# INET-RC/GeoMX

Measured on AMD Instinct MI355X. Metric: samples/sec (whole node), higher is better.
Workload: dtype bf16; 1 GPU; model=geomx_cnn, input=3x224x224, global_batch=512, per_gpu_batch=512, parallelism=dp1, sync_mode=dist_sync, optimizer=sgd_mom

## Files before the change

geomx_amd/csrc/fc.hip:

```cpp

#include <hip/hip_runtime.h>

#include <cstdint>

typedef unsigned short bf16_t;
typedef __attribute__((ext_vector_type(8))) short bf16x8;

#define FC_C 32
#define FC_THREADS 256
#define FC_PERM_HW 128
#define FC_PERM_LD 129

__device__ __forceinline__ bf16_t fc_f2bf(float f) {
  union { float f; unsigned int u; } cv;
  cv.f = f;
  if ((cv.u & 0x7FFFFFFFu) > 0x7F800000u)
    return (bf16_t)((cv.u >> 16) | 0x0040u);
  const unsigned int lsb = (cv.u >> 16) & 1;
  return (bf16_t)((cv.u + 0x7FFFu + lsb) >> 16);
}

__global__ __launch_bounds__(FC_THREADS) void k_fc_w_permute_bf16(
    const float* __restrict__ w, bf16_t* __restrict__ wp, int HW) {
  __shared__ float tile[FC_C * FC_PERM_LD];
  const int t = threadIdx.x;
  const int hw0 = blockIdx.x * FC_PERM_HW;
  const long long o = blockIdx.y;
  const float* src = w + o * FC_C * HW;
  {
    const int hw = t & (FC_PERM_HW - 1), c0 = t >> 7;
    if (hw0 + hw < HW) {
      float v[FC_C / 2];
#pragma unroll
      for (int i = 0; i < FC_C / 2; ++i)
        v[i] = src[(long long)(c0 + 2 * i) * HW + hw0 + hw];
#pragma unroll
      for (int i = 0; i < FC_C / 2; ++i)
        tile[(c0 + 2 * i) * FC_PERM_LD + hw] = v[i];
    }
  }
  __syncthreads();
  bf16_t* dst = wp + o * HW * FC_C;
  const int cg = t & 3;
#pragma unroll
  for (int p = 0; p < FC_PERM_HW / (FC_THREADS / 4); ++p) {
    const int hw = p * (FC_THREADS / 4) + (t >> 2);
    if (hw0 + hw < HW) {
      union { bf16x8 v; bf16_t e[8]; } pk;
#pragma unroll
      for (int j = 0; j < 8; ++j)
        pk.e[j] = fc_f2bf(tile[(cg * 8 + j) * FC_PERM_LD + hw]);
      *reinterpret_cast<bf16x8*>(dst + (long long)(hw0 + hw) * FC_C +
                                 cg * 8) = pk.v;
    }
  }
}

__global__ __launch_bounds__(FC_THREADS) void k_fc_w_unpermute_f32(
    const bf16_t* __restrict__ gp, float* __restrict__ g, int HW) {
  __shared__ float tile[FC_C * FC_PERM_LD];
  const int t = threadIdx.x;
  const int hw0 = blockIdx.x * FC_PERM_HW;
  const long long o = blockIdx.y;
  const bf16_t* src = gp + o * HW * FC_C;
  const int cg = t & 3;
#pragma unroll
  for (int p = 0; p < FC_PERM_HW / (FC_THREADS / 4); ++p) {
    const int hw = p * (FC_THREADS / 4) + (t >> 2);
    if (hw0 + hw < HW) {
      union { bf16x8 v; bf16_t e[8]; } pk;
      pk.v = *reinterpret_cast<const bf16x8*>(
          src + (long long)(hw0 + hw) * FC_C + cg * 8);
#pragma unroll
      for (int j = 0; j < 8; ++j) {
        union { unsigned int u; float f; } cv;
        cv.u = (unsigned int)pk.e[j] << 16;
        tile[(cg * 8 + j) * FC_PERM_LD + hw] = cv.f;
      }
    }
  }
  __syncthreads();
  float* dst = g + o * FC_C * HW;
  const int hw = t & (FC_PERM_HW - 1), c0 = t >> 7;
  if (hw0 + hw < HW) {
#pragma unroll
    for (int i = 0; i < FC_C / 2; ++i)
      dst[(long long)(c0 + 2 * i) * HW + hw0 + hw] =
          tile[(c0 + 2 * i) * FC_PERM_LD + hw];
  }
}

#define FC_FLAT_LD 130
__global__ __launch_bounds__(FC_THREADS) void k_fc_flatten_nchw(
    const bf16_t* __restrict__ x, bf16_t* __restrict__ y, int HW) {
  __shared__ bf16_t tile[FC_C * FC_FLAT_LD];
  const int t = threadIdx.x;
  const int hw0 = blockIdx.x * FC_PERM_HW;
  const long long n = blockIdx.y;
  const bf16_t* src = x + n * HW * FC_C;
  const int cg = t & 3;
#pragma unroll
  for (int p = 0; p < FC_PERM_HW / (FC_THREADS / 4); ++p) {
    const int hw = p * (FC_THREADS / 4) + (t >> 2);
    if (hw0 + hw < HW) {
      union { bf16x8 v; bf16_t e[8]; } pk;
      pk.v = *reinterpret_cast<const bf16x8*>(
          src + (long long)(hw0 + hw) * FC_C + cg * 8);
#pragma unroll
      for (int j = 0; j < 8; ++j)
        tile[(cg * 8 + j) * FC_FLAT_LD + hw] = pk.e[j];
    }
  }
  __syncthreads();
  const int wave = t >> 6, lane = t & 63;
#pragma unroll
  for (int i = 0; i < FC_C / 4; ++i) {
    const int c = wave * (FC_C / 4) + i;
    const long long row = (n * FC_C + c) * HW + hw0;
    const int par = (int)(row & 1);
    const bf16_t* trow = tile + c * FC_FLAT_LD;
    bf16_t* dst = y + row;
    const int e0 = 2 * lane - par, e1 = e0 + 1;
    const bool ok0 = e0 >= 0 && hw0 + e0 < HW;
    const bool ok1 = hw0 + e1 < HW;
    if (ok0 && ok1) {
      const unsigned v = (unsigned)trow[e0] | ((unsigned)trow[e1] << 16);
      *reinterpret_cast<unsigned*>(dst + e0) = v;
    } else if (ok0) {
      dst[e0] = trow[e0];
    } else if (ok1) {
      dst[e1] = trow[e1];
    }
    if (par && lane == 0 && hw0 + FC_PERM_HW - 1 < HW)
      dst[FC_PERM_HW - 1] = trow[FC_PERM_HW - 1];
  }
}

extern "C" {

static bool fc_geometry_ok(long long rows, int C, int HW) {
  return C == FC_C && rows > 0 && rows <= 65535 && HW > 0 &&
         HW <= (1 << 24);
}

int geops_fc_w_permute_bf16(const float* w, bf16_t* wp, int O, int C, int HW,
                            hipStream_t s) {
  if (!fc_geometry_ok(O, C, HW)) return -1;
  hipLaunchKernelGGL(k_fc_w_permute_bf16,
                     dim3((HW + FC_PERM_HW - 1) / FC_PERM_HW, O),
                     dim3(FC_THREADS), 0, s, w, wp, HW);
  return 0;
}

int geops_fc_w_unpermute_f32(const bf16_t* gp, float* g, int O, int C, int HW,
                             hipStream_t s) {
  if (!fc_geometry_ok(O, C, HW)) return -1;
  hipLaunchKernelGGL(k_fc_w_unpermute_f32,
                     dim3((HW + FC_PERM_HW - 1) / FC_PERM_HW, O),
                     dim3(FC_THREADS), 0, s, gp, g, HW);
  return 0;
}

int geops_fc_flatten_nchw(const bf16_t* x, bf16_t* y, int N, int C, int HW,
                          hipStream_t s) {
  if (!fc_geometry_ok(N, C, HW)) return -1;
  hipLaunchKernelGGL(k_fc_flatten_nchw,
                     dim3((HW + FC_PERM_HW - 1) / FC_PERM_HW, N),
                     dim3(FC_THREADS), 0, s, x, y, HW);
  return 0;
}

}
```

geomx_amd/csrc/geops.cpp:

```cpp

#include <torch/extension.h>

#include <ATen/cuda/CUDAContext.h>
#include <hip/hip_runtime.h>

#include <cstdint>

extern "C" {
void geops_quantize_2bit(const float*, float*, uint32_t*, long long, float,
                         hipStream_t);
void geops_dequantize_2bit(const uint32_t*, float*, long long, float,
                           hipStream_t);
void geops_bsc_momentum(const float*, float*, float*, float, long long,
                        hipStream_t);
void geops_bsc_pack(const float*, float*, float*, float*, int*, long long*,
                    float, long long, long long, float, bool, hipStream_t);
void geops_bsc_pull_pack(const float*, float*, int*, long long*, long long,
                         long long, float, hipStream_t);
int geops_bsc_fused(const float*, float*, float*, float*, int*, const float*,
                    unsigned long long*, float, long long, long long, float,
                    hipStream_t);
void geops_bsc_unpack(const float*, const int*, float*, long long, long long,
                      bool, hipStream_t);
void geops_dgt_contribution(const float*, float*, long long, int, int,
                            hipStream_t);
void geops_quantize_4bit(const float*, float*, uint8_t*, float*, long long,
                         int, int, bool, hipStream_t);
void geops_dequantize_4bit(const uint8_t*, const float*, float*, long long,
                           int, hipStream_t);
void geops_sgd_update(float*, const float*, float, float, float, long long,
                      hipStream_t);
void geops_sgd_mom_update(float*, const float*, float*, float, float, float,
                          float, long long, hipStream_t);
void geops_adam_update(float*, const float*, float*, float*, float, float,
                       float, float, float, float, long long, hipStream_t);
void geops_dcasgd_update(float*, const float*, float*, float*, float, float,
                         float, float, float, long long, bool, hipStream_t);
void geops_rmsprop_update(float*, const float*, float*, float, float, float,
                          float, float, long long, hipStream_t);
void geops_adagrad_update(float*, const float*, float*, float, float, float,
                          float, long long, hipStream_t);
void geops_signsgd_update(float*, const float*, float, float, float,
                          long long, hipStream_t);
void geops_signum_update(float*, const float*, float*, float, float, float,
                         float, long long, hipStream_t);
void geops_rsp_merge(const long long*, const long long*, const long long*,
                     const float*, long long*, float*, long long, long long,
                     hipStream_t);
void geops_rsp_scatter(const long long*, const float*, float*, long long,
                       long long, long long, bool, hipStream_t);
void geops_rsp_sgd_update(const long long*, const float*, float*, float,
                          float, float, long long, long long, long long,
                          hipStream_t);
void geops_rsp_sgd_mom_update(const long long*, const float*, float*, float*,
                              float, float, float, float, long long,
                              long long, long long, hipStream_t);
void geops_rsp_adam_update(const long long*, const float*, float*, float*,
                           float*, float, float, float, float, float, float,
                           long long, long long, long long, hipStream_t);
void geops_rsp_adagrad_update(const long long*, const float*, float*, float*,
                              float, float, float, float, long long,
                              long long, long long, hipStream_t);
void geops_relu_maxpool2_fwd(const unsigned short*, unsigned short*, uint8_t*,
                             long long, int, int, int, hipStream_t);
void geops_relu_maxpool2_bwd(const unsigned short*, const uint8_t*,
                             unsigned short*, long long, int, int, int,
                             hipStream_t);
int geops_conv5_nhwc(const unsigned short*, const unsigned short*,
                     const float*, unsigned short*, int, int, int, int, int,
                     int, int, int, hipStream_t);
int geops_conv5_pool_nhwc(const unsigned short*, const unsigned short*,
                          const float*, unsigned short*, uint8_t*, int, int,
                          int, int, int, int, int, hipStream_t);
int geops_conv5_pool_nwg_nhwc(const unsigned short*, const unsigned short*,
                              const float*, unsigned short*, uint8_t*, int,
                              int, int, int, int, int, int, int, hipStream_t);
void geops_pad_ch3to4_nhwc(const void*, unsigned short*, long long, int,
                           hipStream_t);
int geops_conv5_pack_frags(const float*, long long, const long long*,
                           unsigned short*, long long, const long long*,
                           unsigned short*, long long, hipStream_t);
int geops_conv5_wrw16_nhwc(const unsigned short*, const unsigned short*,
                           float*, int, int, int, int, int, int, int, int,
                           hipStream_t);
int geops_conv5_wrw4_nhwc(const unsigned short*, const unsigned short*,
                          float*, int, int, int, int, int, int, int, int,
                          hipStream_t);
int geops_conv5_wrw_unpool_nhwc(const unsigned short*, const unsigned short*,
                                const uint8_t*, float*, int, int, int, int,
                                int, int, int, int, hipStream_t);
int geops_conv5_dgrad_unpool_nhwc(const unsigned short*, const uint8_t*,
                                  const unsigned short*, unsigned short*,
                                  int, int, int, int, int, int, int,
                                  hipStream_t);
int geops_conv5_direct_nhwc(const unsigned short*, const unsigned short*,
                            const float*, unsigned short*, int, int, int, int,
                            int, int, int, hipStream_t);
int geops_conv5_dgrad_nwg_nhwc(const unsigned short*, const uint8_t*,
                               const unsigned short*, unsigned short*, int,
                               int, int, int, int, int, int, int,
                               hipStream_t);
int geops_fc_w_permute_bf16(const float*, unsigned short*, int, int, int,
                            hipStream_t);
int geops_fc_w_unpermute_f32(const unsigned short*, float*, int, int, int,
                             hipStream_t);
int geops_fc_flatten_nchw(const unsigned short*, unsigned short*, int, int,
                          int, hipStream_t);
void geops_tr16_probe(const unsigned short*, unsigned short*, hipStream_t);
void geops_tr16_probe2(const unsigned short*, const int*, unsigned short*,
                       hipStream_t);
}

namespace {

hipStream_t cur_stream() {
  return (hipStream_t)at::cuda::getCurrentCUDAStream().stream();
}

void launch_check(const char* what) {
  const hipError_t e = hipGetLastError();
  TORCH_CHECK(e == hipSuccess, what, ": kernel launch failed: ",
              hipGetErrorString(e));
}

void check_f32(const torch::Tensor& t, const char* name) {
  TORCH_CHECK(t.is_cuda(), name, " must be a GPU tensor");
  TORCH_CHECK(t.is_contiguous(), name, " must be contiguous");
  TORCH_CHECK(t.scalar_type() == torch::kFloat32, name, " must be fp32");
  TORCH_CHECK(((uintptr_t)t.data_ptr() & 15) == 0, name,
              " must be 16-byte aligned");
}

void quantize_2bit(torch::Tensor grad, torch::Tensor residual,
                   torch::Tensor out, double thr) {
  check_f32(grad, "grad");
  check_f32(residual, "residual");
  TORCH_CHECK(out.scalar_type() == torch::kInt32 && out.is_contiguous());
  const long long n = grad.numel();
  TORCH_CHECK(residual.numel() == n);
  TORCH_CHECK(out.numel() == (n + 15) / 16);
  geops_quantize_2bit(grad.data_ptr<float>(), residual.data_ptr<float>(),
                      (uint32_t*)out.data_ptr<int32_t>(), n, (float)thr,
                      cur_stream());
  launch_check("quantize_2bit");
}

void dequantize_2bit(torch::Tensor packed, torch::Tensor out, double thr) {
  check_f32(out, "out");
  TORCH_CHECK(packed.scalar_type() == torch::kInt32 && packed.is_contiguous());
  const long long n = out.numel();
  TORCH_CHECK(packed.numel() >= (n + 15) / 16);
  geops_dequantize_2bit((const uint32_t*)packed.data_ptr<int32_t>(),
                        out.data_ptr<float>(), n, (float)thr, cur_stream());
  launch_check("dequantize_2bit");
}

void bsc_momentum(torch::Tensor g, torch::Tensor u, torch::Tensor v,
                  double mu) {
  check_f32(g, "g"); check_f32(u, "u"); check_f32(v, "v");
  const long long n = g.numel();
  TORCH_CHECK(u.numel() == n && v.numel() == n);
  geops_bsc_momentum(g.data_ptr<float>(), u.data_ptr<float>(),
                     v.data_ptr<float>(), (float)mu, n, cur_stream());
  launch_check("bsc_momentum");
}

torch::Tensor make_workspace(const torch::Tensor& like) {
  return torch::empty({2049}, torch::TensorOptions()
                                  .dtype(torch::kInt64)
                                  .device(like.device()));
}

void bsc_pack(torch::Tensor v, torch::Tensor u, torch::Tensor vals,
              torch::Tensor idx, double boundary, double placeholder) {
  check_f32(v, "v"); check_f32(u, "u"); check_f32(vals, "vals");
  TORCH_CHECK(idx.scalar_type() == torch::kInt32 && idx.is_contiguous());
  TORCH_CHECK(vals.numel() == idx.numel());
  auto ws = make_workspace(v);
  geops_bsc_pack(v.data_ptr<float>(), v.data_ptr<float>(),
                 u.data_ptr<float>(), vals.data_ptr<float>(),
                 idx.data_ptr<int32_t>(), (long long*)ws.data_ptr<int64_t>(),
                 (float)boundary, v.numel(), vals.numel(),
                 (float)placeholder, true, cur_stream());
  launch_check("bsc_pack");
}

bool bsc_compress_fused(torch::Tensor g, torch::Tensor u, torch::Tensor v,
                        torch::Tensor vals, torch::Tensor idx,
                        torch::Tensor boundary, double mu,
                        double placeholder) {
// ... 282 lines not shown
  const int rc = geops_conv5_direct_nhwc(
      (const unsigned short*)in.data_ptr(),
      (const unsigned short*)w_frags.data_ptr(), nullptr,
      (unsigned short*)out.data_ptr(), (int)N, (int)Hi, (int)Wi, (int)Ho,
      (int)Wo, (int)CI, (int)CO, cur_stream());
  TORCH_CHECK(rc == 0, "conv5_direct_nhwc: unsupported geometry CI=", CI,
              " CO=", CO, " Hi=", Hi, " Wi=", Wi);
  launch_check("conv5_direct_nhwc");
}

void conv5_dgrad_nwg_nhwc(torch::Tensor in, torch::Tensor mask,
                          torch::Tensor w_frags, torch::Tensor out,
                          int64_t N, int64_t Hi, int64_t Wi, int64_t Ho,
                          int64_t Wo, int64_t CI, int64_t CO, int64_t n_wg) {
  const bool pooled = mask.defined() && mask.numel() > 0;
  TORCH_CHECK(in.is_cuda() && w_frags.is_cuda() && out.is_cuda());
  TORCH_CHECK(in.scalar_type() == torch::kBFloat16 &&
              w_frags.scalar_type() == torch::kBFloat16 &&
              out.scalar_type() == torch::kBFloat16);
  TORCH_CHECK(Hi >= 10 && Wi >= 10 && n_wg >= 1 && n_wg <= 65536,
              "conv5_dgrad_nwg_nhwc: bad size or n_wg");
  if (pooled) {
    TORCH_CHECK(mask.is_cuda() && mask.scalar_type() == torch::kUInt8);
    TORCH_CHECK(in.numel() == N * ((Hi - 8) / 2) * ((Wi - 8) / 2) * CI &&
                    mask.numel() == in.numel(),
                "conv5_dgrad_nwg_nhwc: pooled gradient / mask size mismatch");
  } else {
    TORCH_CHECK(in.numel() == N * (Hi - 8) * (Wi - 8) * CI,
                "conv5_dgrad_nwg_nhwc: gradient size mismatch");
  }
  TORCH_CHECK(out.numel() == N * Ho * Wo * CO &&
                  w_frags.numel() == 25 * 64 * 8,
              "conv5_dgrad_nwg_nhwc: output / weight size mismatch");
  const int rc = geops_conv5_dgrad_nwg_nhwc(
      (const unsigned short*)in.data_ptr(),
      pooled ? mask.data_ptr<uint8_t>() : nullptr,
      (const unsigned short*)w_frags.data_ptr(),
      (unsigned short*)out.data_ptr(), (int)N, (int)Hi, (int)Wi, (int)Ho,
      (int)Wo, (int)CI, (int)CO, (int)n_wg, cur_stream());
  TORCH_CHECK(rc == 0, "conv5_dgrad_nwg_nhwc: unsupported geometry CI=", CI,
              " CO=", CO, " Hi=", Hi, " Wi=", Wi);
  launch_check("conv5_dgrad_nwg_nhwc");
}


void check_fc_operand(const torch::Tensor& t, torch::ScalarType dtype,
                      int64_t numel, const char* name) {
  TORCH_CHECK(t.is_cuda(), name, " must be a GPU tensor");
  TORCH_CHECK(t.is_contiguous(), name, " must be contiguous");
  TORCH_CHECK(t.scalar_type() == dtype, name, " has the wrong dtype");
  TORCH_CHECK(t.numel() == numel, name, " has ", t.numel(),
              " elements, expected ", numel);
  if (dtype != torch::kFloat32)
    TORCH_CHECK(((uintptr_t)t.data_ptr() & 15) == 0, name,
                " must be 16-byte aligned");
}

torch::Tensor fc_w_permute_bf16(torch::Tensor w, int64_t O, int64_t C,
                                int64_t HW) {
  check_fc_operand(w, torch::kFloat32, O * C * HW, "weight");
  auto wp = torch::empty({O, HW * C}, w.options().dtype(torch::kBFloat16));
  const int rc = geops_fc_w_permute_bf16(
      w.data_ptr<float>(), (unsigned short*)wp.data_ptr(), (int)O, (int)C,
      (int)HW, cur_stream());
  TORCH_CHECK(rc == 0, "fc_w_permute_bf16: unsupported geometry O=", O,
              " C=", C, " HW=", HW);
  launch_check("fc_w_permute_bf16");
  return wp;
}

torch::Tensor fc_w_unpermute_f32(torch::Tensor gp, int64_t O, int64_t C,
                                 int64_t HW) {
  check_fc_operand(gp, torch::kBFloat16, O * C * HW, "permuted gradient");
  auto g = torch::empty({O, C * HW}, gp.options().dtype(torch::kFloat32));
  const int rc = geops_fc_w_unpermute_f32(
      (const unsigned short*)gp.data_ptr(), g.data_ptr<float>(), (int)O,
      (int)C, (int)HW, cur_stream());
  TORCH_CHECK(rc == 0, "fc_w_unpermute_f32: unsupported geometry O=", O,
              " C=", C, " HW=", HW);
  launch_check("fc_w_unpermute_f32");
  return g;
}

torch::Tensor fc_flatten_nchw(torch::Tensor x, int64_t N, int64_t C,
                              int64_t HW) {
  check_fc_operand(x, torch::kBFloat16, N * C * HW, "x");
  auto y = torch::empty({N, C * HW}, x.options());
  const int rc = geops_fc_flatten_nchw(
      (const unsigned short*)x.data_ptr(), (unsigned short*)y.data_ptr(),
      (int)N, (int)C, (int)HW, cur_stream());
  TORCH_CHECK(rc == 0, "fc_flatten_nchw: unsupported geometry N=", N,
              " C=", C, " HW=", HW);
  launch_check("fc_flatten_nchw");
  return y;
}

void pad_ch3to4_nhwc(torch::Tensor in, torch::Tensor out, int64_t npix) {
  TORCH_CHECK(in.is_cuda() && out.is_cuda());
  TORCH_CHECK(out.scalar_type() == torch::kBFloat16);
  const bool fp32 = in.scalar_type() == torch::kFloat32;
  TORCH_CHECK(fp32 || in.scalar_type() == torch::kBFloat16);
  geops_pad_ch3to4_nhwc(in.data_ptr(), (unsigned short*)out.data_ptr(),
                        npix, fp32 ? 1 : 0, cur_stream());
  launch_check("pad_ch3to4_nhwc");
}

std::vector<torch::Tensor> conv5_pack_frags(torch::Tensor weight,
                                            torch::Tensor idx0,
                                            c10::optional<torch::Tensor> idx1) {
  TORCH_CHECK(weight.is_cuda() && weight.is_contiguous() &&
                  weight.scalar_type() == torch::kFloat32,
              "conv5_pack_frags: weight must be contiguous fp32 on the GPU");
  const bool two = idx1.has_value() && idx1->defined();
  auto check_idx = [&](const torch::Tensor& t) {
    TORCH_CHECK(t.is_cuda() && t.is_contiguous() &&
                    t.scalar_type() == torch::kInt64 &&
                    t.device() == weight.device() && t.numel() > 0 &&
                    t.numel() % 8 == 0,
                "conv5_pack_frags: index tables are contiguous int64 on the "
                "weight's device, a multiple of 8 long");
  };
  check_idx(idx0);
  if (two) check_idx(*idx1);
  const auto opts = weight.options().dtype(torch::kBFloat16);
  std::vector<torch::Tensor> out;
  out.push_back(torch::empty({idx0.numel()}, opts));
  if (two) out.push_back(torch::empty({idx1->numel()}, opts));
  const int rc = geops_conv5_pack_frags(
      weight.data_ptr<float>(), (long long)weight.numel(),
      (const long long*)idx0.data_ptr<int64_t>(),
      (unsigned short*)out[0].data_ptr(), (long long)idx0.numel(),
      two ? (const long long*)idx1->data_ptr<int64_t>() : nullptr,
      two ? (unsigned short*)out[1].data_ptr() : nullptr,
      two ? (long long)idx1->numel() : 0LL, cur_stream());
  TORCH_CHECK(rc == 0, "conv5_pack_frags: bad table sizes");
  launch_check("conv5_pack_frags");
  return out;
}

void sgd_update(torch::Tensor w, torch::Tensor g, double lr, double wd,
                double rescale) {
  check_f32(w, "w"); check_f32(g, "g");
  TORCH_CHECK(w.numel() == g.numel());
  geops_sgd_update(w.data_ptr<float>(), g.data_ptr<float>(), (float)lr,
                   (float)wd, (float)rescale, w.numel(), cur_stream());
  launch_check("sgd_update");
}

void sgd_mom_update(torch::Tensor w, torch::Tensor g, torch::Tensor mom,
                    double lr, double momentum, double wd, double rescale) {
  check_f32(w, "w"); check_f32(g, "g"); check_f32(mom, "mom");
  geops_sgd_mom_update(w.data_ptr<float>(), g.data_ptr<float>(),
                       mom.data_ptr<float>(), (float)lr, (float)momentum,
                       (float)wd, (float)rescale, w.numel(), cur_stream());
  launch_check("sgd_mom_update");
}

void adam_update(torch::Tensor w, torch::Tensor g, torch::Tensor m,
                 torch::Tensor v, int64_t t, double lr, double beta1,
                 double beta2, double eps, double wd, double rescale) {
  check_f32(w, "w"); check_f32(g, "g"); check_f32(m, "m"); check_f32(v, "v");
  const double lr_t =
      lr * std::sqrt(1.0 - std::pow(beta2, (double)t)) /
      (1.0 - std::pow(beta1, (double)t));
  geops_adam_update(w.data_ptr<float>(), g.data_ptr<float>(),
                    m.data_ptr<float>(), v.data_ptr<float>(), (float)lr_t,
// ... 116 lines not shown
  launch_check("rsp_scatter");
}

void rsp_sgd_update(torch::Tensor w, torch::Tensor ids, torch::Tensor merged,
                    double lr, double wd, double rescale) {
  check_rsp_rows(w, ids, merged);
  geops_rsp_sgd_update(i64p(ids), merged.data_ptr<float>(),
                       w.data_ptr<float>(), (float)lr, (float)wd,
                       (float)rescale, ids.numel(), w.size(0), w.size(1),
                       cur_stream());
  launch_check("rsp_sgd_update");
}

void rsp_sgd_mom_update(torch::Tensor w, torch::Tensor ids,
                        torch::Tensor merged, torch::Tensor mom, double lr,
                        double momentum, double wd, double rescale) {
  check_rsp_rows(w, ids, merged);
  check_rsp_state(mom, w, "mom");
  geops_rsp_sgd_mom_update(i64p(ids), merged.data_ptr<float>(),
                           w.data_ptr<float>(), mom.data_ptr<float>(),
                           (float)lr, (float)momentum, (float)wd,
                           (float)rescale, ids.numel(), w.size(0), w.size(1),
                           cur_stream());
  launch_check("rsp_sgd_mom_update");
}

void rsp_adam_update(torch::Tensor w, torch::Tensor ids, torch::Tensor merged,
                     torch::Tensor m, torch::Tensor v, int64_t t, double lr,
                     double beta1, double beta2, double eps, double wd,
                     double rescale) {
  check_rsp_rows(w, ids, merged);
  check_rsp_state(m, w, "m"); check_rsp_state(v, w, "v");
  const double lr_t =
      lr * std::sqrt(1.0 - std::pow(beta2, (double)t)) /
      (1.0 - std::pow(beta1, (double)t));
  geops_rsp_adam_update(i64p(ids), merged.data_ptr<float>(),
                        w.data_ptr<float>(), m.data_ptr<float>(),
                        v.data_ptr<float>(), (float)lr_t, (float)beta1,
                        (float)beta2, (float)eps, (float)wd, (float)rescale,
                        ids.numel(), w.size(0), w.size(1), cur_stream());
  launch_check("rsp_adam_update");
}

void rsp_adagrad_update(torch::Tensor w, torch::Tensor ids,
                        torch::Tensor merged, torch::Tensor h, double lr,
                        double eps, double wd, double rescale) {
  check_rsp_rows(w, ids, merged);
  check_rsp_state(h, w, "h");
  geops_rsp_adagrad_update(i64p(ids), merged.data_ptr<float>(),
                           w.data_ptr<float>(), h.data_ptr<float>(),
                           (float)lr, (float)eps, (float)wd, (float)rescale,
                           ids.numel(), w.size(0), w.size(1), cur_stream());
  launch_check("rsp_adagrad_update");
}

}

PYBIND11_MODULE(TORCH_EXTENSION_NAME, m) {
  m.doc() = "geomx_amd gfx950 kernel library";
  m.def("quantize_2bit", &quantize_2bit);
  m.def("dequantize_2bit", &dequantize_2bit);
  m.def("bsc_momentum", &bsc_momentum);
  m.def("bsc_pack", &bsc_pack);
  m.def("bsc_pull_pack", &bsc_pull_pack);
  m.def("bsc_compress_fused", &bsc_compress_fused);
  m.def("bsc_unpack", &bsc_unpack);
  m.def("dgt_contribution", &dgt_contribution);
  m.def("quantize_4bit", &quantize_4bit);
  m.def("dequantize_4bit", &dequantize_4bit);
  m.def("conv5_nhwc", &conv5_nhwc);
  m.def("pad_ch3to4_nhwc", &pad_ch3to4_nhwc);
  m.def("conv5_pack_frags", &conv5_pack_frags, py::arg("weight"),
        py::arg("idx0"), py::arg("idx1") = py::none());
  m.def("conv5_wrw_nhwc", &conv5_wrw_nhwc);
  m.def("conv5_wrw_unpool_nhwc", &conv5_wrw_unpool_nhwc);
  m.def("conv5_dgrad_unpool_nhwc", &conv5_dgrad_unpool_nhwc);
  m.def("conv5_direct_nhwc", &conv5_direct_nhwc);
  m.def("conv5_dgrad_nwg_nhwc", &conv5_dgrad_nwg_nhwc);
  m.def("conv5_pool_nhwc", &conv5_pool_nhwc);
  m.def("conv5_pool_nwg_nhwc", &conv5_pool_nwg_nhwc);
  m.def("fc_w_permute_bf16", &fc_w_permute_bf16);
  m.def("fc_w_unpermute_f32", &fc_w_unpermute_f32);
  m.def("fc_flatten_nchw", &fc_flatten_nchw);
  m.def("tr16_probe2", [](torch::Tensor in, torch::Tensor addr,
                          torch::Tensor out) {
    TORCH_CHECK(in.is_cuda() && addr.is_cuda() && out.is_cuda());
    TORCH_CHECK(in.numel() == 512 && addr.numel() == 64 &&
                out.numel() == 256);
    TORCH_CHECK(addr.scalar_type() == torch::kInt32);
    geops_tr16_probe2((const unsigned short*)in.data_ptr(),
                      addr.data_ptr<int32_t>(),
                      (unsigned short*)out.data_ptr(), cur_stream());
    launch_check("tr16_probe2");
  });
  m.def("tr16_probe", [](torch::Tensor in, torch::Tensor out) {
    TORCH_CHECK(in.is_cuda() && out.is_cuda());
    TORCH_CHECK(in.numel() == 64 && out.numel() == 256);
    geops_tr16_probe((const unsigned short*)in.data_ptr(),
                     (unsigned short*)out.data_ptr(), cur_stream());
    launch_check("tr16_probe");
  });
  m.def("relu_maxpool2_fwd", &relu_maxpool2_fwd);
  m.def("relu_maxpool2_bwd", &relu_maxpool2_bwd);
  m.def("sgd_update", &sgd_update);
  m.def("sgd_mom_update", &sgd_mom_update);
  m.def("adam_update", &adam_update);
  m.def("dcasgd_update", &dcasgd_update);
  m.def("rmsprop_update", &rmsprop_update);
  m.def("adagrad_update", &adagrad_update);
  m.def("signsgd_update", &signsgd_update);
  m.def("signum_update", &signum_update);
  m.def("rsp_merge", &rsp_merge);
  m.def("rsp_scatter", &rsp_scatter);
  m.def("rsp_sgd_update", &rsp_sgd_update);
  m.def("rsp_sgd_mom_update", &rsp_sgd_mom_update);
  m.def("rsp_adam_update", &rsp_adam_update);
  m.def("rsp_adagrad_update", &rsp_adagrad_update);
}
```

geomx_amd/ops/fc.py:

```python

from __future__ import annotations

import torch
import torch.nn.functional as F

from . import native_available

FC_CHANNELS = 32


def supported(C: int, O: int, N: int, HW: int) -> bool:
    return (C == FC_CHANNELS and 0 < O <= 65535 and N > 0
            and 0 < HW <= (1 << 24))


def native_route(x: torch.Tensor, weight: torch.Tensor) -> bool:
    if not (x.is_cuda and x.dim() == 4 and native_available()):
        return False
    if torch.is_autocast_enabled("cuda"):
        if torch.get_autocast_dtype("cuda") != torch.bfloat16 or \
                x.dtype not in (torch.bfloat16, torch.float32):
            return False
    elif x.dtype != torch.bfloat16:
        return False
    N, C, H, W = x.shape
    if not supported(C, weight.shape[0], N, H * W):
        return False
    if weight.dtype != torch.float32 or not weight.is_contiguous() \
            or weight.shape[1] != C * H * W:
        return False
    return x.stride() == (H * W * C, 1, W * C, C)


class _FlattenLinearFn(torch.autograd.Function):

    @staticmethod
    def forward(ctx, x, weight, bias):
        from geomx_amd import _geops
        N, C, H, W = x.shape
        xf = x.detach().to(torch.bfloat16).permute(0, 2, 3, 1) \
            .reshape(N, H * W * C)
        with torch.autocast("cuda", enabled=False):
            y = F.linear(_geops.fc_flatten_nchw(xf, N, C, H * W),
                         weight.detach().to(torch.bfloat16),
                         None if bias is None
                         else bias.detach().to(torch.bfloat16))
        ctx.save_for_backward(xf, weight)
        ctx.geom = (N, C, H, W, weight.shape[0])
        ctx.x_dtype = x.dtype
        ctx.b_dtype = None if bias is None else bias.dtype
        return y

    @staticmethod
    def backward(ctx, grad_out):
        from geomx_amd import _geops
        xf, weight = ctx.saved_tensors
        N, C, H, W, O = ctx.geom
        dy = grad_out.to(torch.bfloat16).contiguous()
        grad_x = grad_w = grad_b = None
        if ctx.needs_input_grad[0]:
            wp = _geops.fc_w_permute_bf16(weight.detach(), O, C, H * W)
            grad_x = torch.mm(dy, wp).view(N, H, W, C).permute(0, 3, 1, 2) \
                .to(ctx.x_dtype)
        if ctx.needs_input_grad[1]:
            grad_w = _geops.fc_w_unpermute_f32(torch.mm(dy.t(), xf), O, C,
                                               H * W)
        if ctx.b_dtype is not None and ctx.needs_input_grad[2]:
            grad_b = dy.sum(0).to(ctx.b_dtype)
        return grad_x, grad_w, grad_b


class GeoFlattenLinear(torch.nn.Linear):

    def forward(self, x):
        if native_route(x, self.weight):
            return _FlattenLinearFn.apply(x, self.weight, self.bias)
        return F.linear(torch.flatten(x, 1), self.weight, self.bias)
```

geomx_amd/parallel/trainer.py:

```python

from __future__ import annotations


from typing import Dict, List, Optional

import torch
import torch.distributed as dist

from .. import comm, ops
from ..config import Config
from ..kvstore.optimizer import OptimizerSpec, ServerOptimizer
from ..kvstore.wan import TokenBucket, cross_party_bytes
from ..topology import Topology


class _Bucket:
    __slots__ = ("params", "flat", "param_flat", "views", "ready", "expected",
                 "work", "index", "bsc_u", "bsc_v", "dgt", "res2bit",
                 "wan_buf", "wan_work", "wan_ready")

    def __init__(self, index: int):
        self.index = index
        self.params: List[torch.nn.Parameter] = []
        self.flat: Optional[torch.Tensor] = None
        self.param_flat: Optional[torch.Tensor] = None
        self.views: List[torch.Tensor] = []
        self.ready = 0
        self.expected = 0
        self.work = None
        self.bsc_u: Optional[torch.Tensor] = None
        self.bsc_v: Optional[torch.Tensor] = None
        self.dgt = None
        self.res2bit: Optional[torch.Tensor] = None
        self.wan_buf: Optional[torch.Tensor] = None
        self.wan_work = None
        self.wan_ready = 0.0


class _Bf16Work:

    def __init__(self, work, h, flat):
        self.work = work
        self.h = h
        self.flat = flat

    def wait(self):
        self.work.wait()
        self.flat.copy_(self.h.float())


def _alias_view(flat: torch.Tensor, off: int, p: torch.Tensor) -> torch.Tensor:
    n = p.numel()
    if p.dim() == 4 and p.is_contiguous(memory_format=torch.channels_last) \
            and not p.is_contiguous():
        N, C, H, W = p.shape
        return flat[off:off + n].as_strided((N, C, H, W),
                                            (C * H * W, 1, W * C, C))
    return flat[off:off + n].view(p.shape)


class GeoTrainer:
    def __init__(self, model: torch.nn.Module, cfg: Config, topo: Topology,
                 optimizer: Optional[OptimizerSpec] = None,
                 mode: str = "flat"):
        if mode not in ("flat", "hips"):
            raise ValueError(mode)
        self.model = model
        self.cfg = cfg
        self.topo = topo
        self.mode = mode if topo.world_size > 1 else "flat"
        self.wan = TokenBucket(cfg.wan_rate_for(topo.party_id),
                               rtt_ms=cfg.wan_rtt_ms)
        self.device = topo.device
        self.spec = optimizer or OptimizerSpec(name="sgd", lr=0.01)
        self.server_opt = ServerOptimizer(self.spec)
        self._step = 0
        self._ts = None
        if (cfg.enable_ts and self.mode == "hips"
                and topo.num_parties > 1 and topo.is_leader
                and cfg.mode == "dist_sync"):
            from ..kvstore.tsengine import TSExchange
            self._ts = TSExchange(topo.leader_group, topo.party_id,
                                  topo.leader_ranks, wan=self.wan)
        if (cfg.mode == "dist_async" and self.mode == "hips"
                and topo.num_parties > 1
                and cfg.compression not in (None, "fp16")):
            raise ValueError(
                f"compression {cfg.compression!r} is not supported in the "
                "pipelined dist_async WAN tier; use dist_sync or "
                "compression in (None, 'fp16')")
        self._build_buckets()
        self._register_hooks()

    def _build_buckets(self):
        params = [p for p in self.model.parameters() if p.requires_grad]
        params = params[::-1]
        cap = self.cfg.bucket_mb * 1024 * 1024 // 4
        self.buckets: List[_Bucket] = []
        cur = _Bucket(0)
        size = 0
        for p in params:
            n = p.numel()
            if size > 0 and size + n > cap:
                self.buckets.append(cur)
                cur = _Bucket(len(self.buckets))
                size = 0
            cur.params.append(p)
            size += n
        if cur.params:
            self.buckets.append(cur)
        self.param_bucket: Dict[torch.nn.Parameter, tuple] = {}
        ALIGN = 64

        def aligned(n):
            return (n + ALIGN - 1) // ALIGN * ALIGN

        for b in self.buckets:
            total = sum(aligned(p.numel()) for p in b.params)
            b.flat = torch.zeros(total, dtype=torch.float32, device=self.device)
            b.expected = len(b.params)
            b.param_flat = torch.zeros(total, dtype=torch.float32,
                                       device=self.device)
            off = 0
            for p in b.params:
                n = p.numel()
                view = _alias_view(b.flat, off, p)
                b.views.append(view)
                p.grad = view
                pview = _alias_view(b.param_flat, off, p)
                with torch.no_grad():
                    pview.copy_(p.data.float())
                p.data = pview
                self.param_bucket[p] = (b, len(b.views) - 1)
                off += aligned(n)

    def _register_hooks(self):
        self._hook_handles = []
        for p in self.param_bucket:
            h = p.register_post_accumulate_grad_hook(self._on_grad_ready)
            self._hook_handles.append(h)

    def _on_grad_ready(self, p: torch.nn.Parameter):
        b, _ = self.param_bucket[p]
        b.ready += 1
        if b.ready == b.expected:
            self._launch_bucket(b)

    def _launch_bucket(self, b: _Bucket):
        if self.topo.world_size == 1:
            return
        if self.mode == "flat":
            b.flat.div_(self.topo.world_size)
            if self.cfg.comm_dtype == "bf16":
                h = b.flat.to(torch.bfloat16)
                work = comm.all_reduce(h, async_op=True)
                b.work = _Bf16Work(work, h, b.flat)
            else:
                b.work = comm.all_reduce(b.flat, async_op=True)
        else:
            b.flat.div_(self.topo.num_all_workers)
            b.work = comm.all_reduce(b.flat, group=self.topo.party_group,
                                     async_op=True)

    def step(self, lr: Optional[float] = None,
             batch_size: Optional[int] = None):
        self._step += 1
        if self.mode == "hips" and self.topo.num_parties > 1 \
                and self.cfg.mode == "dist_async" \
                and self.cfg.compression in (None, "fp16"):
            self._wait_buckets()
            self._wan_tier_async()
            return
        self.allreduce_grads()
        self.update(batch_size=batch_size, lr=lr)

    def _wait_buckets(self):
        for b in self.buckets:
            if b.work is not None:
                b.work.wait()
                b.work = None

    def allreduce_grads(self):
        self._wait_buckets()
        if self.mode == "hips" and self.topo.num_parties > 1:
            self._wan_tier()
        elif self.mode == "flat" and self.wan.enabled \
                and self.cfg.num_parties > 1:
            for b in self.buckets:
                self.wan.charge(cross_party_bytes(
                    "all_reduce", b.flat.numel() * 4, self.cfg.num_parties))

    def update(self, batch_size: Optional[int] = None,
               lr: Optional[float] = None):
        if lr is not None:
            self.spec.lr = lr
        rs = None if batch_size is None \
            else self.spec.rescale_grad / batch_size
        for b in self.buckets:
            self.server_opt.update(("bucket", b.index), b.param_flat,
                                   b.flat, rescale=rs)
            b.ready = 0

    def _wan_tier_async(self):
        topo = self.topo
        P = topo.num_parties
        ctype = self.cfg.compression
        for b in self.buckets:
            if b.wan_work is not None or b.wan_ready:
                if b.wan_work is not None:
                    b.wan_work.wait()
                    b.wan_work = None
                self.wan.wait_until(b.wan_ready)
                apply_buf = b.wan_buf
                if ctype == "fp16":
                    apply_buf = b.wan_buf.float()
                if topo.num_workers > 1:
                    comm.broadcast(apply_buf, src=topo.leader_rank,
                                   group=topo.party_group)
                self.server_opt.update(("bucket", b.index), b.param_flat,
                                       apply_buf)
            if topo.is_leader:
                if ctype == "fp16":
                    snap = b.flat.to(torch.float16)
                    nbytes = snap.numel() * 2
                else:
                    snap = b.flat.clone()
                    nbytes = snap.numel() * 4
                b.wan_buf = snap
                b.wan_work = comm.all_reduce(snap, group=topo.leader_group,
                                             async_op=True)
                b.wan_ready = self.wan.charge_async(
                    cross_party_bytes("all_reduce", nbytes, P))
            else:
                if b.wan_buf is None or b.wan_buf.numel() != b.flat.numel():
                    b.wan_buf = torch.empty_like(b.flat)
                if ctype == "fp16":
                    b.wan_buf = torch.empty(b.flat.numel(),
                                            dtype=torch.float16,
                                            device=b.flat.device)
                b.wan_ready = 1e-9
            b.ready = 0

    def _wan_tier(self):
        topo = self.topo
        P = topo.num_parties
        ctype = self.cfg.compression
        for b in self.buckets:
            if topo.is_leader:
                small = b.flat.numel() < self.cfg.size_lower_bound
                if ctype in ("bsc", "bsc_dgt", "mpq") and small:
                    if ctype == "mpq":
                        h = b.flat.to(torch.float16)
                        comm.all_reduce(h, group=topo.leader_group)
                        self.wan.charge(cross_party_bytes(
                            "all_reduce", h.numel() * 2, P))
                        b.flat.copy_(h.float())
                    else:
                        comm.all_reduce(b.flat, group=topo.leader_group)
                        self.wan.charge(cross_party_bytes(
                            "all_reduce", b.flat.numel() * 4, P))
                elif ctype == "bsc_dgt":
                    if b.bsc_u is None:
                        b.bsc_u = torch.zeros_like(b.flat)
                        b.bsc_v = torch.zeros_like(b.flat)
                    vals, idx = ops.bsc_compress(b.flat, b.bsc_u, b.bsc_v,
                                                 self.cfg.bsc_ratio)
                    if b.dgt is None or b.dgt.numel != vals.numel():
                        from ..kvstore.dgt import DGTState
                        b.dgt = DGTState(vals.numel(), vals.device,
                                         chunk_elems=max(
                                             64, self.cfg.dgt_block_size // 4),
                                         k=self.cfg.dgt_k,
                                         alpha=self.cfg.dgt_alpha, mode=3)
                    vals = vals.masked_fill(idx < 0, 0.0)
                    b.dgt.residual.zero_()
                    payload = b.dgt.compress(vals) + (idx,)
                    gathered = [[torch.empty_like(t) for _ in range(P)]
                                for t in payload]
                    for lst, t in zip(gathered, payload):
                        comm.all_gather(lst, t, group=topo.leader_group)
                    self.wan.charge(cross_party_bytes(
                        "all_gather",
                        b.dgt.wire_bytes() + idx.numel() * 4, P))
                    acc = torch.zeros_like(b.flat)
                    for p_ in range(P):
                        v_p = b.dgt.decompress(
                            *(lst[p_] for lst in gathered[:4]))
                        ops.bsc_decompress(v_p, gathered[4][p_],
                                           b.flat.numel(), out=acc,
                                           accumulate=True)
                    b.flat.copy_(acc)
                elif ctype == "bsc" or ctype == "mpq":
                    if b.bsc_u is None:
                        b.bsc_u = torch.zeros_like(b.flat)
                        b.bsc_v = torch.zeros_like(b.flat)
                    vals, idx = ops.bsc_compress(b.flat, b.bsc_u, b.bsc_v,
                                                 self.cfg.bsc_ratio)
                    vlist = [torch.empty_like(vals) for _ in range(P)]
                    ilist = [torch.empty_like(idx) for _ in range(P)]
                    comm.all_gather(vlist, vals, group=topo.leader_group)
                    comm.all_gather(ilist, idx, group=topo.leader_group)
                    self.wan.charge(cross_party_bytes(
                        "all_gather", vals.numel() * 8, P))
                    acc = torch.zeros_like(b.flat)
                    for v_, i_ in zip(vlist, ilist):
                        ops.bsc_decompress(v_, i_, b.flat.numel(),
                                           out=acc, accumulate=True)
                    b.flat.copy_(acc)
                elif ctype == "dgt":
                    if b.dgt is None:
                        from ..kvstore.dgt import DGTState
                        b.dgt = DGTState(b.flat.numel(), b.flat.device,
                                         chunk_elems=max(
                                             64, self.cfg.dgt_block_size // 4),
                                         k=self.cfg.dgt_k,
                                         alpha=self.cfg.dgt_alpha,
                                         mode=self.cfg.enable_dgt or 3)
                    if b.dgt.mode >= 3:
                        payload = b.dgt.compress(b.flat)
                        gathered = [[torch.empty_like(t) for _ in range(P)]
                                    for t in payload]
                        for lst, t in zip(gathered, payload):
                            comm.all_gather(lst, t, group=topo.leader_group)
                        self.wan.charge(cross_party_bytes(
                            "all_gather", b.dgt.wire_bytes(), P))
                        acc = torch.zeros_like(b.flat)
                        for p_ in range(P):
                            acc += b.dgt.decompress(
                                *(lst[p_] for lst in gathered))
                        b.flat.copy_(acc)
                    else:
                        lossy, wire = b.dgt.transform(b.flat)
                        b.flat.copy_(lossy)
                        comm.all_reduce(b.flat, group=topo.leader_group)
                        self.wan.charge(cross_party_bytes(
                            "all_reduce", wire, P))
                elif ctype == "2bit":
                    if b.res2bit is None:
                        b.res2bit = torch.zeros_like(b.flat)
                    thr = self.cfg.threshold
                    packed = ops.quantize_2bit(b.flat, b.res2bit, thr)
                    plist = [torch.empty_like(packed) for _ in range(P)]
                    comm.all_gather(plist, packed, group=topo.leader_group)
                    self.wan.charge(cross_party_bytes(
                        "all_gather", packed.numel() * 4, P))
                    acc = torch.zeros_like(b.flat)
                    tmp = torch.empty_like(b.flat)
                    for p_ in plist:
                        ops.dequantize_2bit(p_, b.flat.numel(), thr, out=tmp)
                        acc += tmp
                    b.flat.copy_(acc)
                elif ctype in ("fp16", "mpq"):
                    if self._ts is not None:
                        b.flat.copy_(self._ts.allreduce_sum(
                            b.flat, wire_dtype=torch.float16))
                    else:
                        h = b.flat.to(torch.float16)
                        comm.all_reduce(h, group=topo.leader_group)
                        self.wan.charge(cross_party_bytes(
                            "all_reduce", h.numel() * 2, P))
                        b.flat.copy_(h.float())
                elif self._ts is not None:
                    b.flat.copy_(self._ts.allreduce_sum(b.flat))
                else:
                    comm.all_reduce(b.flat, group=topo.leader_group)
                    self.wan.charge(cross_party_bytes(
                        "all_reduce", b.flat.numel() * 4, P))
            if topo.num_workers > 1:
                comm.broadcast(b.flat, src=topo.leader_rank,
                               group=topo.party_group)

    @property
    def learning_rate(self) -> float:
        return self.server_opt.spec.lr

    def set_learning_rate(self, lr: float) -> None:
        self.server_opt.set_learning_rate(lr)

    def zero_grad(self):
        for b in self.buckets:
            b.flat.zero_()
            b.ready = 0

    def refresh_params(self):
        ALIGN = 64
        for b in self.buckets:
            off = 0
            for p in b.params:
                n = p.numel()
                pv = _alias_view(b.param_flat, off, p)
                if p.data.data_ptr() != pv.data_ptr():
                    with torch.no_grad():
                        pv.copy_(p.data.float())
                    p.data = pv
                off += (n + ALIGN - 1) // ALIGN * ALIGN

    def save_optimizer_states(self, fname: str, dump_optimizer: bool = False):
        import pickle
        with open(fname, "wb") as f:
            pickle.dump(self.server_opt.state_dict(), f)

    def load_optimizer_states(self, fname: str):
        import pickle
        with open(fname, "rb") as f:
            self.server_opt.load_state_dict(pickle.load(f),
                                            device=self.device)
```

Before: 282,600 samples/s.

## Fuse FC weight bf16 packing and write FC weight grads directly into bucket

A new kernel produces both the row-major bf16 weight and the permuted bf16 weight in one pass over the fp32 weight during forward, so backward no longer re-reads and re-permutes the weight. A grad-sink mechanism lets the FC backward unpermute its weight gradient straight into the trainer's flat gradient bucket, and zero_grad skips zeroing those sink regions. This removes a separate cast, a permute, a gradient copy and part of the bucket memset, at the cost of more trainer bookkeeping around grad settlement and holding the permuted weight across forward and backward.

```diff
diff --git a/geomx_amd/csrc/fc.hip b/geomx_amd/csrc/fc.hip
--- a/geomx_amd/csrc/fc.hip
+++ b/geomx_amd/csrc/fc.hip
@@ -56,7 +56,70 @@
   }
 }
 
-__global__ __launch_bounds__(FC_THREADS) void k_fc_w_unpermute_f32(
+__global__ __launch_bounds__(FC_THREADS) void k_fc_w_pack2_bf16(
+    const float* __restrict__ w, bf16_t* __restrict__ wb,
+    bf16_t* __restrict__ wp, int HW) {
+  __shared__ float tile[FC_C * FC_PERM_LD];
+  const int t = threadIdx.x;
+  const int hw0 = blockIdx.x * FC_PERM_HW;
+  const long long o = blockIdx.y;
+  const float* src = w + o * FC_C * HW;
+  {
+    const int hw = t & (FC_PERM_HW - 1), c0 = t >> 7;
+    if (hw0 + hw < HW) {
+      float v[FC_C / 2];
+#pragma unroll
+      for (int i = 0; i < FC_C / 2; ++i)
+        v[i] = src[(long long)(c0 + 2 * i) * HW + hw0 + hw];
+#pragma unroll
+      for (int i = 0; i < FC_C / 2; ++i)
+        tile[(c0 + 2 * i) * FC_PERM_LD + hw] = v[i];
+    }
+  }
+  __syncthreads();
+  if (wp != nullptr) {
+    bf16_t* dst = wp + o * HW * FC_C;
+    const int cg = t & 3;
+#pragma unroll
+    for (int p = 0; p < FC_PERM_HW / (FC_THREADS / 4); ++p) {
+      const int hw = p * (FC_THREADS / 4) + (t >> 2);
+      if (hw0 + hw < HW) {
+        union { bf16x8 v; bf16_t e[8]; } pk;
+#pragma unroll
+        for (int j = 0; j < 8; ++j)
+          pk.e[j] = fc_f2bf(tile[(cg * 8 + j) * FC_PERM_LD + hw]);
+        *reinterpret_cast<bf16x8*>(dst + (long long)(hw0 + hw) * FC_C +
+                                   cg * 8) = pk.v;
+      }
+    }
+  }
+  const int wave = t >> 6, lane = t & 63;
+#pragma unroll
+  for (int i = 0; i < FC_C / 4; ++i) {
+    const int c = wave * (FC_C / 4) + i;
+    const long long row = (o * FC_C + c) * HW + hw0;
+    const int par = (int)(row & 1);
+    const float* trow = tile + c * FC_PERM_LD;
+    bf16_t* dst = wb + row;
+    const int e0 = 2 * lane - par, e1 = e0 + 1;
+    const bool ok0 = e0 >= 0 && hw0 + e0 < HW;
+    const bool ok1 = hw0 + e1 < HW;
+    if (ok0 && ok1) {
+      const unsigned v = (unsigned)fc_f2bf(trow[e0]) |
+                         ((unsigned)fc_f2bf(trow[e1]) << 16);
+      *reinterpret_cast<unsigned*>(dst + e0) = v;
+    } else if (ok0) {
+      dst[e0] = fc_f2bf(trow[e0]);
+    } else if (ok1) {
+      dst[e1] = fc_f2bf(trow[e1]);
+    }
+    if (par && lane == 0 && hw0 + FC_PERM_HW - 1 < HW)
+      dst[FC_PERM_HW - 1] = fc_f2bf(trow[FC_PERM_HW - 1]);
+  }
+}
+
+template <bool kPosZero>
+__device__ __forceinline__ void fc_w_unpermute_body(
     const bf16_t* __restrict__ gp, float* __restrict__ g, int HW) {
   __shared__ float tile[FC_C * FC_PERM_LD];
   const int t = threadIdx.x;
@@ -84,10 +147,21 @@
   const int hw = t & (FC_PERM_HW - 1), c0 = t >> 7;
   if (hw0 + hw < HW) {
 #pragma unroll
-    for (int i = 0; i < FC_C / 2; ++i)
-      dst[(long long)(c0 + 2 * i) * HW + hw0 + hw] =
-          tile[(c0 + 2 * i) * FC_PERM_LD + hw];
-  }
+    for (int i = 0; i < FC_C / 2; ++i) {
+      const float v = tile[(c0 + 2 * i) * FC_PERM_LD + hw];
+      dst[(long long)(c0 + 2 * i) * HW + hw0 + hw] = kPosZero ? v + 0.0f : v;
+    }
+  }
+}
+
+__global__ __launch_bounds__(FC_THREADS) void k_fc_w_unpermute_f32(
+    const bf16_t* __restrict__ gp, float* __restrict__ g, int HW) {
+  fc_w_unpermute_body<false>(gp, g, HW);
+}
+
+__global__ __launch_bounds__(FC_THREADS) void k_fc_w_unpermute_into(
+    const bf16_t* __restrict__ gp, float* __restrict__ g, int HW) {
+  fc_w_unpermute_body<true>(gp, g, HW);
 }
 
 #define FC_FLAT_LD 130
@@ -161,6 +235,24 @@
   return 0;
 }
 
+int geops_fc_w_pack2_bf16(const float* w, bf16_t* wb, bf16_t* wp, int O,
+                          int C, int HW, hipStream_t s) {
+  if (!fc_geometry_ok(O, C, HW)) return -1;
+  hipLaunchKernelGGL(k_fc_w_pack2_bf16,
+                     dim3((HW + FC_PERM_HW - 1) / FC_PERM_HW, O),
+                     dim3(FC_THREADS), 0, s, w, wb, wp, HW);
+  return 0;
+}
+
+int geops_fc_w_unpermute_into(const bf16_t* gp, float* g, int O, int C,
+                              int HW, hipStream_t s) {
+  if (!fc_geometry_ok(O, C, HW)) return -1;
+  hipLaunchKernelGGL(k_fc_w_unpermute_into,
+                     dim3((HW + FC_PERM_HW - 1) / FC_PERM_HW, O),
+                     dim3(FC_THREADS), 0, s, gp, g, HW);
+  return 0;
+}
+
 int geops_fc_flatten_nchw(const bf16_t* x, bf16_t* y, int N, int C, int HW,
                           hipStream_t s) {
   if (!fc_geometry_ok(N, C, HW)) return -1;
diff --git a/geomx_amd/csrc/geops.cpp b/geomx_amd/csrc/geops.cpp
--- a/geomx_amd/csrc/geops.cpp
+++ b/geomx_amd/csrc/geops.cpp
@@ -106,6 +106,10 @@
                              hipStream_t);
 int geops_fc_flatten_nchw(const unsigned short*, unsigned short*, int, int,
                           int, hipStream_t);
+int geops_fc_w_pack2_bf16(const float*, unsigned short*, unsigned short*,
+                          int, int, int, hipStream_t);
+int geops_fc_w_unpermute_into(const unsigned short*, float*, int, int, int,
+                              hipStream_t);
 void geops_tr16_probe(const unsigned short*, unsigned short*, hipStream_t);
 void geops_tr16_probe2(const unsigned short*, const int*, unsigned short*,
                        hipStream_t);
@@ -554,6 +558,70 @@
   return g;
 }
 
+void check_on_current_device(const torch::Tensor& t, const char* name) {
+  TORCH_CHECK(t.get_device() == at::cuda::current_device(), name,
+              " is on device ", t.get_device(),
+              ", the current device is ", (int)at::cuda::current_device());
+}
+
+std::tuple<torch::Tensor, c10::optional<torch::Tensor>> fc_w_pack2_bf16(
+    torch::Tensor w, int64_t O, int64_t C, int64_t HW, bool want_perm,
+    c10::optional<torch::Tensor> wb_out,
+    c10::optional<torch::Tensor> wp_out) {
+  check_fc_operand(w, torch::kFloat32, O * C * HW, "weight");
+  check_on_current_device(w, "weight");
+  const auto opts = w.options().dtype(torch::kBFloat16);
+  torch::Tensor wb;
+  if (wb_out.has_value()) {
+    wb = *wb_out;
+    TORCH_CHECK(wb.is_cuda() && wb.is_contiguous() &&
+                    wb.scalar_type() == torch::kBFloat16 &&
+                    wb.numel() == O * C * HW,
+                "wb_out must be a contiguous GPU bf16 tensor of ",
+                O * C * HW, " elements");
+    TORCH_CHECK(((uintptr_t)wb.data_ptr() & 3) == 0,
+                "wb_out must be 4-byte aligned");
+    TORCH_CHECK(wb.device() == w.device(),
+                "wb_out must be on the weight's device");
+  } else {
+    wb = torch::empty({O, C * HW}, opts);
+  }
+  c10::optional<torch::Tensor> wp;
+  if (want_perm) {
+    if (wp_out.has_value()) {
+      check_fc_operand(*wp_out, torch::kBFloat16, O * C * HW, "wp_out");
+      TORCH_CHECK(wp_out->device() == w.device(),
+                  "wp_out must be on the weight's device");
+      wp = *wp_out;
+    } else {
+      wp = torch::empty({O, HW * C}, opts);
+    }
+  }
+  const int rc = geops_fc_w_pack2_bf16(
+      w.data_ptr<float>(), (unsigned short*)wb.data_ptr(),
+      wp.has_value() ? (unsigned short*)wp->data_ptr() : nullptr, (int)O,
+      (int)C, (int)HW, cur_stream());
+  TORCH_CHECK(rc == 0, "fc_w_pack2_bf16: unsupported geometry O=", O,
+              " C=", C, " HW=", HW);
+  launch_check("fc_w_pack2_bf16");
+  return {wb, wp};
+}
+
+void fc_w_unpermute_into(torch::Tensor gp, torch::Tensor dst, int64_t O,
+                         int64_t C, int64_t HW) {
+  check_fc_operand(gp, torch::kBFloat16, O * C * HW, "permuted gradient");
+  check_fc_operand(dst, torch::kFloat32, O * C * HW, "destination");
+  TORCH_CHECK(dst.device() == gp.device(),
+              "destination must be on the permuted gradient's device");
+  check_on_current_device(gp, "permuted gradient");
+  const int rc = geops_fc_w_unpermute_into(
+      (const unsigned short*)gp.data_ptr(), dst.data_ptr<float>(), (int)O,
+      (int)C, (int)HW, cur_stream());
+  TORCH_CHECK(rc == 0, "fc_w_unpermute_into: unsupported geometry O=", O,
+              " C=", C, " HW=", HW);
+  launch_check("fc_w_unpermute_into");
+}
+
 torch::Tensor fc_flatten_nchw(torch::Tensor x, int64_t N, int64_t C,
                               int64_t HW) {
   check_fc_operand(x, torch::kBFloat16, N * C * HW, "x");
@@ -836,6 +904,10 @@
   m.def("fc_w_permute_bf16", &fc_w_permute_bf16);
   m.def("fc_w_unpermute_f32", &fc_w_unpermute_f32);
   m.def("fc_flatten_nchw", &fc_flatten_nchw);
+  m.def("fc_w_pack2_bf16", &fc_w_pack2_bf16, py::arg("w"), py::arg("O"),
+        py::arg("C"), py::arg("HW"), py::arg("want_perm"),
+        py::arg("wb_out") = py::none(), py::arg("wp_out") = py::none());
+  m.def("fc_w_unpermute_into", &fc_w_unpermute_into);
   m.def("tr16_probe2", [](torch::Tensor in, torch::Tensor addr,
                           torch::Tensor out) {
     TORCH_CHECK(in.is_cuda() && addr.is_cuda() && out.is_cuda());
diff --git a/geomx_amd/gradsink.py b/geomx_amd/gradsink.py
--- /dev/null
+++ b/geomx_amd/gradsink.py
@@ -0,0 +1,61 @@
+
+from __future__ import annotations
+
+import weakref
+from typing import Optional
+
+import torch
+
+_ATTR = "_geo_grad_sink"
+
+
+class GradSink:
+
+    __slots__ = ("_flat", "_off", "_size", "_stride", "_armed", "_param")
+
+    def __init__(self, flat: torch.Tensor, view: torch.Tensor,
+                 param: torch.Tensor):
+        self._param = weakref.ref(param)
+        self._flat = flat
+        self._off = view.storage_offset() - flat.storage_offset()
+        self._size = tuple(view.shape)
+        self._stride = tuple(view.stride())
+        self._armed = False
+
+    def view(self) -> torch.Tensor:
+        return self._flat.as_strided(self._size, self._stride,
+                                     self._flat.storage_offset() + self._off)
+
+    def data_ptr(self) -> int:
+        return self._flat.data_ptr() + 4 * self._off
+
+    def arm(self) -> None:
+        self._armed = True
+
+    @property
+    def armed(self) -> bool:
+        return self._armed
+
+    def disarm(self) -> None:
+        self._armed = False
+
+    def take(self) -> Optional[torch.Tensor]:
+        p = self._param()
+        if not self._armed or p is None or p.grad is not None:
+            self._armed = False
+            return None
+        self._armed = False
+        return self.view()
+
+
+def attach(p: torch.Tensor, sink: GradSink) -> None:
+    setattr(p, _ATTR, sink)
+
+
+def detach(p: torch.Tensor) -> None:
+    if hasattr(p, _ATTR):
+        delattr(p, _ATTR)
+
+
+def sink_of(p: torch.Tensor) -> Optional[GradSink]:
+    return getattr(p, _ATTR, None)
diff --git a/geomx_amd/ops/fc.py b/geomx_amd/ops/fc.py
--- a/geomx_amd/ops/fc.py
+++ b/geomx_amd/ops/fc.py
@@ -4,6 +4,7 @@
 import torch
 import torch.nn.functional as F
 
+from .. import gradsink
 from . import native_available
 
 FC_CHANNELS = 32
@@ -40,12 +41,15 @@
         N, C, H, W = x.shape
         xf = x.detach().to(torch.bfloat16).permute(0, 2, 3, 1) \
             .reshape(N, H * W * C)
+        wb, wp = _geops.fc_w_pack2_bf16(weight.detach(), weight.shape[0],
+                                        C, H * W, ctx.needs_input_grad[0])
         with torch.autocast("cuda", enabled=False):
-            y = F.linear(_geops.fc_flatten_nchw(xf, N, C, H * W),
-                         weight.detach().to(torch.bfloat16),
+            y = F.linear(_geops.fc_flatten_nchw(xf, N, C, H * W), wb,
                          None if bias is None
                          else bias.detach().to(torch.bfloat16))
-        ctx.save_for_backward(xf, weight)
+        ctx.save_for_backward(xf)
+        ctx.wp = wp
+        ctx.sink = gradsink.sink_of(weight)
         ctx.geom = (N, C, H, W, weight.shape[0])
         ctx.x_dtype = x.dtype
         ctx.b_dtype = None if bias is None else bias.dtype
@@ -54,17 +58,20 @@
     @staticmethod
     def backward(ctx, grad_out):
         from geomx_amd import _geops
-        xf, weight = ctx.saved_tensors
+        xf, = ctx.saved_tensors
         N, C, H, W, O = ctx.geom
         dy = grad_out.to(torch.bfloat16).contiguous()
         grad_x = grad_w = grad_b = None
         if ctx.needs_input_grad[0]:
-            wp = _geops.fc_w_permute_bf16(weight.detach(), O, C, H * W)
-            grad_x = torch.mm(dy, wp).view(N, H, W, C).permute(0, 3, 1, 2) \
+            grad_x = torch.mm(dy, ctx.wp).view(N, H, W, C).permute(0, 3, 1, 2) \
                 .to(ctx.x_dtype)
         if ctx.needs_input_grad[1]:
-            grad_w = _geops.fc_w_unpermute_f32(torch.mm(dy.t(), xf), O, C,
-                                               H * W)
+            gp = torch.mm(dy.t(), xf)
+            grad_w = None if ctx.sink is None else ctx.sink.take()
+            if grad_w is not None:
+                _geops.fc_w_unpermute_into(gp, grad_w, O, C, H * W)
+            else:
+                grad_w = _geops.fc_w_unpermute_f32(gp, O, C, H * W)
         if ctx.b_dtype is not None and ctx.needs_input_grad[2]:
             grad_b = dy.sum(0).to(ctx.b_dtype)
         return grad_x, grad_w, grad_b
@@ -72,6 +79,9 @@
 
 class GeoFlattenLinear(torch.nn.Linear):
 
+    def grad_sink_parameters(self):
+        return (self.weight,)
+
     def forward(self, x):
         if native_route(x, self.weight):
             return _FlattenLinearFn.apply(x, self.weight, self.bias)
diff --git a/geomx_amd/parallel/trainer.py b/geomx_amd/parallel/trainer.py
--- a/geomx_amd/parallel/trainer.py
+++ b/geomx_amd/parallel/trainer.py
@@ -7,7 +7,7 @@
 import torch
 import torch.distributed as dist
 
-from .. import comm, ops
+from .. import comm, gradsink, ops
 from ..config import Config
 from ..kvstore.optimizer import OptimizerSpec, ServerOptimizer
 from ..kvstore.wan import TokenBucket, cross_party_bytes
@@ -17,7 +17,7 @@
 class _Bucket:
     __slots__ = ("params", "flat", "param_flat", "views", "ready", "expected",
                  "work", "index", "bsc_u", "bsc_v", "dgt", "res2bit",
-                 "wan_buf", "wan_work", "wan_ready")
+                 "wan_buf", "wan_work", "wan_ready", "clear")
 
     def __init__(self, index: int):
         self.index = index
@@ -25,6 +25,7 @@
         self.flat: Optional[torch.Tensor] = None
         self.param_flat: Optional[torch.Tensor] = None
         self.views: List[torch.Tensor] = []
+        self.clear: List[torch.Tensor] = []
         self.ready = 0
         self.expected = 0
         self.work = None
@@ -62,10 +63,12 @@
 class GeoTrainer:
     def __init__(self, model: torch.nn.Module, cfg: Config, topo: Topology,
                  optimizer: Optional[OptimizerSpec] = None,
-                 mode: str = "flat"):
+                 mode: str = "flat", grad_sinks: bool = True):
         if mode not in ("flat", "hips"):
             raise ValueError(mode)
         self.model = model
+        self._use_sinks = grad_sinks
+        self._settled = False
         self.cfg = cfg
         self.topo = topo
         self.mode = mode if topo.world_size > 1 else "flat"
@@ -115,6 +118,14 @@
         def aligned(n):
             return (n + ALIGN - 1) // ALIGN * ALIGN
 
+        sinkable = set()
+        if self._use_sinks:
+            for m in self.model.modules():
+                offer = getattr(m, "grad_sink_parameters", None)
+                if offer is not None:
+                    sinkable.update(id(p) for p in offer())
+        self.sinks: Dict[torch.nn.Parameter, gradsink.GradSink] = {}
+
         for b in self.buckets:
             total = sum(aligned(p.numel()) for p in b.params)
             b.flat = torch.zeros(total, dtype=torch.float32, device=self.device)
@@ -122,6 +133,7 @@
             b.param_flat = torch.zeros(total, dtype=torch.float32,
                                        device=self.device)
             off = 0
+            lo = 0
             for p in b.params:
                 n = p.numel()
                 view = _alias_view(b.flat, off, p)
@@ -132,7 +144,17 @@
                     pview.copy_(p.data.float())
                 p.data = pview
                 self.param_bucket[p] = (b, len(b.views) - 1)
+                gradsink.detach(p)
+                if id(p) in sinkable:
+                    sink = gradsink.GradSink(b.flat, view, p)
+                    gradsink.attach(p, sink)
+                    self.sinks[p] = sink
+                    if off > lo:
+                        b.clear.append(b.flat[lo:off])
+                    lo = off + n
                 off += aligned(n)
+            if total > lo:
+                b.clear.append(b.flat[lo:total])
 
     def _register_hooks(self):
         self._hook_handles = []
@@ -141,7 +163,19 @@
             self._hook_handles.append(h)
 
     def _on_grad_ready(self, p: torch.nn.Parameter):
-        b, _ = self.param_bucket[p]
+        b, i = self.param_bucket[p]
+        view = b.views[i]
+        g = p.grad
+        if g is not None and (g.data_ptr() != view.data_ptr()
+                              or g.dtype != view.dtype
+                              or g.stride() != view.stride()):
+            with torch.no_grad():
+                view.copy_(g)
+            p.grad = view
+        sink = self.sinks.get(p)
+        if sink is not None:
+            sink.disarm()
+        self._settled = False
         b.ready += 1
         if b.ready == b.expected:
             self._launch_bucket(b)
@@ -174,7 +208,19 @@
         self.allreduce_grads()
         self.update(batch_size=batch_size, lr=lr)
 
+    def _settle_grads(self):
+        if self._settled:
+            return
+        for p, (b, i) in self.param_bucket.items():
+            if p.grad is None:
+                b.views[i].zero_()
+                p.grad = b.views[i]
+        for sink in self.sinks.values():
+            sink.disarm()
+        self._settled = True
+
     def _wait_buckets(self):
+        self._settle_grads()
         for b in self.buckets:
             if b.work is not None:
                 b.work.wait()
@@ -196,10 +242,12 @@
             self.spec.lr = lr
         rs = None if batch_size is None \
             else self.spec.rescale_grad / batch_size
+        self._settle_grads()
         for b in self.buckets:
             self.server_opt.update(("bucket", b.index), b.param_flat,
                                    b.flat, rescale=rs)
             b.ready = 0
+        self._settled = False
 
     def _wan_tier_async(self):
         topo = self.topo
@@ -240,6 +288,7 @@
                                             device=b.flat.device)
                 b.wan_ready = 1e-9
             b.ready = 0
+        self._settled = False
 
     def _wan_tier(self):
         topo = self.topo
@@ -379,8 +428,13 @@
 
     def zero_grad(self):
         for b in self.buckets:
-            b.flat.zero_()
+            for r in b.clear:
+                r.zero_()
             b.ready = 0
+        for p, sink in self.sinks.items():
+            p.grad = None
+            sink.arm()
+        self._settled = False
 
     def refresh_params(self):
         ALIGN = 64
```

Result: faster. 300,200 samples/s (median of 6 runs) (+6.2%).
